# articulatory/articulatory

Measured on AMD Instinct MI355X. Metric: audio samples/sec (16 kHz) EMA->wav HiFi-CAR, batch 64, higher is better.
Workload: dtype fp32; 1 GPU; configs[2]: HiFi-CAR (e2w_hifigan_car.yaml generator) 13-dim pitch+EMA -> 16 kHz, batch 64/GPU, 10 s clips, 80 sequential chunks of 25 frames; batch_per_gpu=64, frames=2000, chunk_frames=25, weights=synthetic seed 1234 (articulatory_amd.utils.synth), parallelism=utterance-sharded x1, arithmetic=exact fp32 products (v_mfma_f32_32x32x2_f32), fp32 accumulate, gather=none

## Files before the change

articulatory_amd/csrc/hificar.hip:

```cpp
#include "hificar_kernels.hip.h"
#include "hificar_launch.h"
#include "hificar_backward.hip.h"
#include "hificar_disc_kernels.hip.h"
#include "hificar_bigru_kernels.hip.h"

#include "../../include/hificar.h"

#include <algorithm>
#include <queue>
#include <cmath>
#include <cstdarg>
#include <cstdio>
#include <cstring>
#include <functional>
#include <map>
#include <string>
#include <vector>

using namespace hificar;

static thread_local char g_err[1024] = "";

static int fail(int code, const char* fmt, ...) {
    va_list ap;
// ... 41 lines not shown
    int scale = 1;
    int cin = 0, cout = 0;
};

struct PlanKey {
    const ConvLayer* layers[6];
    int nseq, rows, zrep;
    int flags;
    bool operator<(const PlanKey& o) const { return memcmp(this, &o, sizeof(PlanKey)) < 0; }
};

struct ConvPlan {
    ConvShape shape;
    unsigned grid = 0;
    size_t lds = 0;
    std::string name;
    MultiConvParams conv = {};
    PairParams pair = {};
};

struct hificar_handle {
    hificar_config cfg;
    int arch = 0;
    std::vector<GBlockLayers> gb;
    int c_last = 0;
    bool finalized = false;
    int precision = HIFICAR_PREC_F32;
    bool profile_detail = false;
    bool use_pair = true;
    double mi1_penalty = 1.05;
    int pick_throughput = 0;
    bool pair_small = true;
    int ksplit = 1;
    int cf = 0;
    int cin_pad = 0;
    int hop = 1;
    int num_cus = 256;
    std::map<std::string, std::vector<int64_t>> expected;
    std::map<std::string, HostTensor> tensors;
    ConvLayer input_conv;
    std::vector<ConvLayer> ups;
    std::vector<ConvLayer> convs1;
    std::vector<ConvLayer> convs2;
    float* d_out_w = nullptr;
    float out_bias = 0.f;
    float* d_out_bias = nullptr;
    void* train = nullptr;
    void (*train_free)(hificar_handle*) = nullptr;
    float* d_mlp_w[5] = {nullptr, nullptr, nullptr, nullptr, nullptr};
    float* d_mlp_b[5] = {nullptr, nullptr, nullptr, nullptr, nullptr};
    float* d_spk_emb = nullptr;
    float* d_spk_w = nullptr;
    float* d_spk_b = nullptr;
    float* d_ph_emb = nullptr;
    float* d_phfc_w = nullptr;
    float* d_phfc_b = nullptr;
    std::vector<void*> allocs;
    char* d_zeros = nullptr;
    void* d_tab = nullptr;
    void* h_tab = nullptr;
    size_t tab_bytes = 0;
    hipEvent_t tab_copied = nullptr;
    struct StepSlot {
        hipEvent_t done = nullptr;
        bool used = false;
    };
// ... 27 lines not shown
    bool shared_chip = false;
    int ar_dual_min = 17, ar_dual_max = 62;
    hipStream_t ar_side = nullptr;
    hipEvent_t ar_ev[2] = {nullptr, nullptr};
    unsigned long long sched_up_seq = 0;
    hipEvent_t done_ev = nullptr;
    bool done_valid = false;
    hipStream_t done_stream = nullptr;
    struct Tap {
        float* dst;
        size_t cap;
    };
    std::map<std::string, Tap> taps;
    float* tap_scratch = nullptr;
    size_t tap_scratch_elems = 0;
    bool profiling = false;
    struct ProfRec {
        hipEvent_t e0, e1;
        std::string name;
        double flops, bytes;
    };
    std::vector<ProfRec> prof;
    hipStream_t prof_stream = nullptr;
};

static FILE* g_launch_log = nullptr;
static void read_env_switches(hificar_handle* h) {
    if (const char* e = getenv("HIFICAR_PROFILE_DETAIL")) h->profile_detail = atoi(e) != 0;
    if (const char* e = getenv("HIFICAR_LAUNCH_LOG")) {
        if (!g_launch_log && *e) g_launch_log = fopen(e, "a");
        if (g_launch_log) h->profile_detail = true;
    }
    if (const char* e = getenv("HIFICAR_KSPLIT")) h->ksplit = atoi(e);
    if (const char* e = getenv("HIFICAR_PAIR")) h->use_pair = atoi(e) != 0;
    if (const char* e = getenv("HIFICAR_PAIR_SMALL")) h->pair_small = atoi(e) != 0;
    if (const char* e = getenv("HIFICAR_AR_DUAL_MIN")) h->ar_dual_min = atoi(e);
    if (const char* e = getenv("HIFICAR_AR_DUAL_MAX")) h->ar_dual_max = atoi(e);
}

struct ProfScope {
    hificar_handle* h;
    hipStream_t s;
    hipEvent_t e0 = nullptr, e1 = nullptr;
    std::string name;
    double flops, bytes;
    ProfScope(hificar_handle* h_, hipStream_t s_, const std::string& n, double f, double b) : h(h_), s(s_), flops(f), bytes(b) {
        if (g_launch_log) {
            fprintf(g_launch_log, "%s\t%.0f\t%.0f\n", n.c_str(), f, b);
            fflush(g_launch_log);
        }
        if (!h->profiling) return;
        name = n;
        (void)hipEventCreate(&e0);
        (void)hipEventCreate(&e1);
        (void)hipEventRecord(e0, s);
    }
    ~ProfScope() {
        if (!h->profiling) return;
        (void)hipEventRecord(e1, s);
        h->prof.push_back({e0, e1, name, flops, bytes});
        h->prof_stream = s;
    }
};

static size_t round_up_sz(size_t x, size_t m) { return (x + m - 1) / m * m; }
static int arena_add(hificar_handle* h, size_t min_bytes);
// ... 708 lines not shown
        for (int t : lists[w]) tiles[pos++] = t;
    }
    start[G] = pos;
    *d_start = reinterpret_cast<int*>(a.d + a.used);
    *d_tiles = *d_start + n_start;
    a.used += take;
    HIP_TRY(hipMemcpyAsync(const_cast<int*>(*d_start), start, bytes, hipMemcpyHostToDevice, stream));
    ++h->sched_up_seq;
    return HIFICAR_OK;
}

static int enter_stream(hificar_handle* h, hipStream_t stream) {
    if (h->have_last_stream && h->last_stream != stream) {
        if (h->done_valid && h->done_stream == h->last_stream) {
            HIP_TRY(hipStreamWaitEvent(stream, h->done_ev, 0));
        } else {
            if (!h->xstream_ev) HIP_TRY(hipEventCreateWithFlags(&h->xstream_ev, hipEventDisableTiming));
            HIP_TRY(hipEventRecord(h->xstream_ev, h->last_stream));
            HIP_TRY(hipStreamWaitEvent(stream, h->xstream_ev, 0));
        }
    }
    h->done_valid = false;
    h->last_stream = stream;
    h->have_last_stream = true;
    return HIFICAR_OK;
}

struct TileCfg {
    int MI, WM, WN;
    int KS;
    int NB;
};
static size_t out_buf_bytes(const TileCfg& t) { return (size_t)t.KS * (t.WM * t.MI * 32) * (t.WN * t.NB * 32 + 4) * sizeof(float); }
constexpr int kNumTileCfgs = 15;
static const TileCfg kTileCfgs[kNumTileCfgs] = {{4, 1, 4, 1, 1}, {4, 2, 2, 1, 1}, {4, 4, 1, 1, 1}, {2, 2, 2, 1, 2}, {2, 4, 1, 1, 2},
                                                {2, 1, 4, 1, 2}, {2, 1, 4, 1, 1}, {2, 2, 2, 1, 1}, {2, 4, 1, 1, 1},
                                                {1, 1, 4, 1, 1}, {1, 2, 2, 1, 1}, {1, 4, 1, 1, 1}, {4, 1, 1, 4, 1}, {2, 1, 1, 4, 1}, {1, 1, 1, 4, 1}};

struct ConvIO {
    const char* xs;
    const float* res;
    float* y;
    char* ys;
    const float* mask_src = nullptr;
    float mask_slope = 0.f;
    long long x_seq_bytes = 0;
    int x_row_bytes = 0;
    int x_rows = 0;
    int x_up = 0;
    float x_slope = -1.f;
    const float* x_more[3] = {nullptr, nullptr, nullptr};
    int x_n = 1;
};

struct ConvRep {
    int n = 1;
    long long zs_x = 0, zs_w = 0, zs_y = 0, zs_b = 0;
};

static TileCfg pick_tile(const hificar_handle* h, const ConvLayer* const* layers, int nbr, int nseq, int rows, int zrep) {
    const ConvLayer& L0 = *layers[0];
    const bool f32 = h->precision == HIFICAR_PREC_F32;
    int halo_all = 0;
    for (int b = 0; b < nbr; ++b) halo_all = std::max(halo_all, layers[b]->off_max - layers[b]->off_min);
    TileCfg tc = {1, 4, 1, 1, 1};
    double best = 1e300;
    int nsteps_min = 1 << 30;
    for (int b = 0; b < nbr; ++b) nsteps_min = std::min(nsteps_min, layers[b]->ntaps * (L0.chunk16 / 16));
    for (int ti = 0; ti < kNumTileCfgs; ++ti) {
        const TileCfg& t = kTileCfgs[ti];
        const int TM = t.WM * t.MI * 32;
        const int chunk = L0.chunk16, RB = chunk * 4;
        if (t.NB == 2 && (f32 || L0.chunk16 == 16)) continue;
        const size_t obuf = (f32 && t.KS == 1) ? 0 : out_buf_bytes(t);
        if (2 * round_up_sz((size_t)(TM + halo_all) * RB, 1024) + obuf > 160 * 1024) continue;
        if (t.NB == 2) {
            bool ok = L0.n_blocks32 >= 2;
            for (int b = 0; b < nbr; ++b) ok = ok && (layers[b]->n_phase == 1 || layers[b]->nb32_per_phase % 2 == 0);
            if (!ok) continue;
        }
        if (t.KS == 4 && (h->ksplit == 0 || nsteps_min < 2)) continue;
        if (t.KS == 1 && h->ksplit == 2 && nsteps_min >= 2) continue;
        const long long tiles_per_branch = (long long)nseq * ((rows + TM - 1) / TM) * ((L0.n_blocks32 + t.WN * t.NB - 1) / (t.WN * t.NB));
        const long long total = tiles_per_branch * nbr * zrep;
        const int G = (int)std::min<long long>(total, h->num_cus);
        const int nchunks = L0.cin_pad / chunk;
        double total_cost = 0.0, heaviest = 0.0, lightest = 1e300, cb[3] = {0.0, 0.0, 0.0};
        for (int b = 0; b < nbr; ++b) {
            const double slab = f32 ? 8 * 64.0 : 3 * 32 / 0.75;
            double c = (double)layers[b]->ntaps * (L0.cin_pad / 16) * slab * t.MI * t.NB + 2500.0 + 400.0 * nchunks;
            if (t.KS == 4) {
                const int steps = layers[b]->ntaps * (chunk / 16);
                c = (double)((steps + 3) / 4) * nchunks * slab * t.MI + 4000.0 + 600.0 * nchunks;
            }
            total_cost += c * tiles_per_branch * zrep;
            heaviest = std::max(heaviest, c);
            lightest = std::min(lightest, c);
            cb[b] = c;
        }
        double worst = std::max(heaviest, total_cost / G);
        if (!h->shared_chip && total > G && total <= 4096) {
            std::sort(cb, cb + nbr, [](double x, double y) { return x > y; });
            std::priority_queue<double, std::vector<double>, std::greater<double>> load;
            for (int w = 0; w < G; ++w) load.push(0.0);
            worst = 0.0;
            for (int b = 0; b < nbr; ++b)
                for (long long i = 0; i < tiles_per_branch * zrep; ++i) {
                    const double v = load.top() + cb[b];
                    load.pop();
                    load.push(v);
                    worst = std::max(worst, v);
                }
        } else if (total % G != 0) {
            worst = std::max(worst, total_cost / G + 0.5 * lightest);
        }
        if (h->pick_throughput > 0 && total >= h->pick_throughput) worst = total_cost / h->num_cus;
        if (t.NB == 2) worst *= f32 ? (t.MI == 4 ? 0.95 : t.MI == 2 ? 0.975 : 1.02) : (t.MI == 2 ? 0.93 : 1.10);
        else if (t.MI < 4) worst *= f32 ? (t.MI == 2 ? 1.02 : h->mi1_penalty) : (t.MI == 2 ? 1.10 : 1.25);
        if (t.KS == 4) worst *= 1.05;
        if (worst < best * 0.98) {
            best = worst;
            tc = t;
        }
    }
    return tc;
}

static std::string plan_name(const hificar_handle* h, const ConvShape& s, const ConvLayer& L0, int nbr) {
    static const char* const family[] = {"conv_f32do_kernel", "conv_bf16x3_kernel", "conv_bf16x3nb_kernel", "conv_sk_f32_kernel", "conv_sk_bf16x3_kernel",
                                         "conv_pair_f32_kernel", "conv_pair_bf16x3_kernel"};
    char kname[96];
    int n = s.family == kConvSkF32 || s.family == kConvSkBf16x3 ? snprintf(kname, sizeof(kname), "%s<%d,%d>", family[s.family], s.mi, s.nc16)
                                                                : snprintf(kname, sizeof(kname), "%s<%d,%d,%d,%d>", family[s.family], s.mi, s.wm, s.wn, s.nc16);
    if (h->profile_detail) snprintf(kname + n, sizeof(kname) - n, "|%s x%d", L0.name.c_str(), nbr);
    return kname;
}

static int build_conv_plan(hificar_handle* h, const ConvLayer* const* layers, int nbr, int nseq, int rows, int zrep, hipStream_t stream, ConvPlan& pl) {
    const ConvLayer& L0 = *layers[0];
    const bool f32 = h->precision == HIFICAR_PREC_F32;
    MultiConvParams& mp = pl.conv;
    const TileCfg tc = pick_tile(h, layers, nbr, nseq, rows, zrep);
    int halo_all = 0;
    for (int b = 0; b < nbr; ++b) halo_all = std::max(halo_all, layers[b]->off_max - layers[b]->off_min);
    const int TM = tc.WM * tc.MI * 32, nc16 = L0.chunk16 / 16;
    const size_t buf_bytes = round_up_sz((size_t)(TM + halo_all) * L0.chunk16 * 4, 1024);
    const bool dout = f32 && tc.KS == 1;
    pl.shape = {dout ? kConvF32do : tc.KS == 4 ? (f32 ? kConvSkF32 : kConvSkBf16x3) : tc.NB == 2 ? kConvBf16x3nb : kConvBf16x3, tc.MI, tc.WM, tc.WN, nc16};
    pl.lds = 2 * buf_bytes + (dout ? 0 : out_buf_bytes(tc));
    mp.buf_bytes = (int)buf_bytes;
    mp.n_branches = nbr;
    mp.nseq_tiles = nseq * ((rows + TM - 1) / TM);
    mp.ngroups = (L0.n_blocks32 + tc.WN * tc.NB - 1) / (tc.WN * tc.NB);
    mp.total_tiles = nbr * zrep * mp.ngroups * mp.nseq_tiles;
    pl.grid = (unsigned)std::min(mp.total_tiles, h->num_cus);
    {
        double wbytes = 0.0;
        for (int b = 0; b < nbr; ++b) wbytes += 4.0 * layers[b]->cin_pad * layers[b]->cout_total * layers[b]->ntaps * zrep;
        const double abytes = 4.0 * nseq * rows * L0.cin_pad * nbr * zrep;
        mp.xcd_order = (mp.total_tiles <= h->num_cus && mp.total_tiles >= 16 && wbytes > 2.0 * abytes) ? 1 : 0;
    }
    mp.stage_cached = mp.ngroups > 2 ? 1 : 0;
    pl.name = plan_name(h, pl.shape, L0, nbr);
    TileLists lists;
    if (mp.total_tiles <= h->num_cus && nbr == 1 && zrep == 1 && mp.ngroups >= 2 && mp.nseq_tiles >= 8 && !h->shared_chip &&
        4.0 * L0.cin_pad * L0.cout_total * L0.ntaps > 6.0e6)
        lists = xcd_block_lists(mp.nseq_tiles, mp.ngroups, h->num_cus);
    if (!lists.empty()) {
        pl.grid = (unsigned)lists.size();
        mp.xcd_order = 0;
    } else if (mp.total_tiles > (int)pl.grid) {
        std::vector<double> costs((size_t)mp.total_tiles);
        const int tpb = mp.ngroups * mp.nseq_tiles * zrep;
        for (int b = 0; b < nbr; ++b)
            for (int i = 0; i < tpb; ++i) costs[(size_t)b * tpb + i] = layers[b]->ntaps + 1.0;
        lists = lpt_lists(costs, (int)pl.grid);
    }
    return lists.empty() ? HIFICAR_OK : upload_schedule(h, lists, mp.total_tiles, stream, &mp.sched_start, &mp.sched_tiles);
}

struct PairIOB {
    const float* xf;
    const char* xs;
    const float* res;
    float* y;
    char* ys;
};

static bool pair_small_tiles(const hificar_handle* h, int C, int k2, int nseq, int rows) {
    if (!h->pair_small || h->ksplit == 0 || C != 32 || h->precision != HIFICAR_PREC_F32 || nseq <= 0 || (long long)nseq * rows < 8000) return false;
    const int tmo = 4 * 4 * 32 - (k2 - 1);
    return 3LL * nseq * ((rows + tmo - 1) / tmo) < h->num_cus;
}

static bool pair_eligible(const hificar_handle* h, const ConvLayer& a, const ConvLayer& b, int nseq = 0, int rows = 0) {
    if (!(h->use_pair && a.d_w16c && b.d_w16c && a.d_w32c && b.d_w32c && a.cin == b.cin && a.ntaps >= 2 &&
          b.ntaps >= 2 && b.dilation == 1 && a.K == b.K))
        return false;
// ... 17 lines not shown
    const int C = l1[0]->cin;
    bool small = true;
    for (int b = 0; b < nbr; ++b) small = small && pair_small_tiles(h, C, l2[b]->ntaps, nseq, rows);
    const int MI = small ? 1 : 4, WM = C == 64 ? 2 : 4;
    const int TMc = WM * MI * 32, RB = C * 4;
    const bool f32 = h->precision == HIFICAR_PREC_F32;
    PairParams& pp = pl.pair;
    int halo_max = 0, tile = 0;
    for (int b = 0; b < nbr; ++b) {
        halo_max = std::max(halo_max, l1[b]->off_max - l1[b]->off_min);
        const int tmo = TMc - (l2[b]->ntaps - 1);
        pp.tiles_per_seq[b] = (rows + tmo - 1) / tmo;
        pp.tile_start[b] = tile;
        tile += nseq * pp.tiles_per_seq[b];
    }
    pp.tile_start[nbr] = tile;
    pp.n_branches = nbr;
    pp.nseq = nseq;
    pp.in_bytes = (int)round_up_sz((size_t)(TMc + halo_max) * RB, 1024);
    pp.ts_bytes = (int)std::max<size_t>((size_t)(TMc + 16) * RB, (size_t)TMc * (C + 4) * sizeof(float));
    pl.lds = (size_t)pp.in_bytes + pp.ts_bytes;
    if (pl.lds > 160 * 1024) return fail(HIFICAR_E_INVALID, "internal: pair kernel LDS too large (%zu)", pl.lds);
    pl.grid = (unsigned)std::min(tile, h->num_cus);
    pl.shape = {f32 ? kPairF32 : kPairBf16x3, MI, WM, 4 / WM, C / 16};
    pl.name = plan_name(h, pl.shape, *l1[0], nbr);
    if (tile <= (int)pl.grid) return HIFICAR_OK;
    std::vector<double> costs((size_t)tile);
    for (int b = 0; b < nbr; ++b)
        for (int i = pp.tile_start[b]; i < pp.tile_start[b + 1]; ++i) costs[i] = l1[b]->ntaps + l2[b]->ntaps + 2.0;
    return upload_schedule(h, lpt_lists(costs, (int)pl.grid), tile, stream, &pp.sched_start, &pp.sched_tiles);
}

static const ConvPlan* get_plan(hificar_handle* h, const ConvLayer* const* a, const ConvLayer* const* b, int nbr, int nseq, int rows, int zrep,
                                hipStream_t stream, int* rc) {
    *rc = HIFICAR_OK;
    PlanKey k = {{}, nseq, rows, zrep, (h->precision == HIFICAR_PREC_F32 ? 1 : 0) | (h->train ? 2 : 0) | (h->shared_chip ? 4 : 0) | (b ? 8 : 0)};
    for (int i = 0; i < nbr; ++i) k.layers[i] = a[i];
    for (int i = 0; b && i < nbr; ++i) k.layers[3 + i] = b[i];
    auto it = h->plans.find(k);
    if (it == h->plans.end()) {
        ConvPlan pl;
        if (h->plans.size() > 20000) *rc = evict_plans(h);
        if (*rc == HIFICAR_OK)
            *rc = b ? build_pair_plan(h, a, b, nbr, nseq, rows, stream, pl) : build_conv_plan(h, a, nbr, nseq, rows, zrep, stream, pl);
        if (*rc != HIFICAR_OK) return nullptr;
        it = h->plans.emplace(k, std::move(pl)).first;
    }
    return &it->second;
}

static int launch_conv(hificar_handle* h, const ConvLayer* const* layers, int nbr, int nseq, int rows, const ConvIO* io,
                              float slope_out, const Ragged& rg, hipStream_t stream, const ConvRep& zr = ConvRep()) {
    int rc;
    const ConvPlan* const pl = get_plan(h, layers, nullptr, nbr, nseq, rows, zr.n, stream, &rc);
    if (!pl) return rc;
    const int TM = pl->shape.wm * pl->shape.mi * 32;
    const ConvLayer& L0 = *layers[0];
    const bool f32 = h->precision == HIFICAR_PREC_F32;
    MultiConvParams mp = pl->conv;
    double flops = 0.0, bytes = 0.0;
    for (int b = 0; b < nbr; ++b) {
        const ConvLayer& Lb = *layers[b];
        if (Lb.n_blocks32 != L0.n_blocks32 || Lb.chunk16 != L0.chunk16 || Lb.cin_pad != L0.cin_pad)
            return fail(HIFICAR_E_INVALID, "internal: branch shape mismatch");
        fill_params(mp.p[b], Lb, rows, TM, io[b].res, io[b].y, rg);
        mp.p[b].xs = io[b].xs;
        mp.p[b].ys = io[b].ys;
        if (io[b].x_slope >= 0.f) {
            if (!f32) return fail(HIFICAR_E_INVALID, "internal: pre-activation input rows of %s outside the exact-fp32 layer-by-layer launches", Lb.name.c_str());
            if (io[b].x_n < 1 || io[b].x_n > 4) return fail(HIFICAR_E_INVALID, "internal: %d input streams of %s", io[b].x_n, Lb.name.c_str());
            mp.p[b].act_in = io[b].x_n;
            for (int q = 0; q + 1 < io[b].x_n; ++q) mp.p[b].xs_more[q] = reinterpret_cast<const char*>(io[b].x_more[q]);
            mp.p[b].slope_in = io[b].x_slope;
        }
        mp.p[b].mask_src = io[b].mask_src;
        mp.p[b].mask_slope = io[b].mask_slope;
        mp.p[b].x_seq_bytes = io[b].x_seq_bytes;
        mp.p[b].x_row_bytes = io[b].x_row_bytes;
        mp.p[b].x_rows = io[b].x_rows;
        if (io[b].x_up > 1) {
            if (rows % io[b].x_up != 0 || io[b].x_seq_bytes != 0 || io[b].x_row_bytes != 0)
                return fail(HIFICAR_E_INVALID, "internal: upsampled input rows of %s", Lb.name.c_str());
            mp.p[b].x_up = io[b].x_up;
            mp.p[b].x_up_rcp = (unsigned)(0x100000000ull / (unsigned)io[b].x_up) + 1u;
            mp.p[b].x_seq_bytes = (long long)(rows / io[b].x_up) * Lb.cin_pad * 4;
        }
        mp.p[b].zeros = h->d_zeros;
        mp.p[b].slope_out = slope_out;
        mp.p[b].cout_real = Lb.cout_pad;
        if (f32) mp.p[b].w16 = reinterpret_cast<const bf16x8*>(Lb.d_w32);
        const double pos = (double)nseq * rows;
        flops += 2.0 * pos * Lb.cin * Lb.cout * Lb.K * zr.n;
        bytes += 4.0 * (pos * Lb.cin_pad * (io[b].x_slope >= 0.f ? io[b].x_n : 1) / std::max(1, io[b].x_up) + pos * Lb.cout_total * ((io[b].res ? 1 : 0) + (io[b].y ? 1 : 0) + (io[b].ys ? 1 : 0)) +
                        (double)Lb.cin * Lb.cout * Lb.K);
    }
    mp.zrep = zr.n;
    mp.zs_x = zr.zs_x;
    mp.zs_w = zr.zs_w;
    mp.zs_y = zr.zs_y;
    mp.zs_b = zr.zs_b;
    ProfScope prof(h, stream, pl->name, flops, bytes);
    const hipError_t e = conv_launch(pl->shape, &mp, dim3(pl->grid, 1, 1), pl->lds, stream);
    if (e != hipSuccess) return fail(HIFICAR_E_HIP, "conv launch (%s, %s) failed: %s", L0.name.c_str(), pl->name.c_str(), hipGetErrorString(e));
    return HIFICAR_OK;
}

static int launch_pair(hificar_handle* h, const ConvLayer* const* l1, const ConvLayer* const* l2, int nbr, int nseq, int rows,
                              const PairIOB* io, float slope, const Ragged& rg, hipStream_t stream) {
    int rc;
    const ConvPlan* const pl = get_plan(h, l1, l2, nbr, nseq, rows, 1, stream, &rc);
    if (!pl) return rc;
    const int TMc = pl->shape.wm * pl->shape.mi * 32;
    const int C = l1[0]->cin;
    const bool f32 = h->precision == HIFICAR_PREC_F32;
    PairParams pp = pl->pair;
    double flops = 0.0, bytes = 0.0;
    for (int b = 0; b < nbr; ++b) {
        const ConvLayer& A = *l1[b];
        const ConvLayer& B = *l2[b];
        fill_params(pp.p1[b], A, rows, TMc, nullptr, nullptr, rg);
        fill_params(pp.p2[b], B, rows, TMc, io[b].res, io[b].y, rg);
        pp.p1[b].w16 = f32 ? reinterpret_cast<const bf16x8*>(A.d_w32c) : reinterpret_cast<const bf16x8*>(A.d_w16c);
        pp.p2[b].w16 = f32 ? reinterpret_cast<const bf16x8*>(B.d_w32c) : reinterpret_cast<const bf16x8*>(B.d_w16c);
        pp.p1[b].xs = io[b].xs;
        pp.p1[b].xf = io[b].xf;
        pp.p1[b].slope_in = slope;
        pp.p1[b].zeros = h->d_zeros;
// ... 183 lines not shown
        if (cfg.use_ar && (rc = emit_tap(h, "ar_feats", ws.xin, f32 ? h->cin_pad : -h->cin_pad, h->cf, cfg.ar_output, B, 1, f32 ? 0 : 1, stream, T)) != HIFICAR_OK)
            return rc;
    }
    const size_t tap_se = tapping ? stage_elems(h, B, T) : 0;
    const int nbk = cfg.n_blocks;
    int order[kMaxBlk];
    for (int j = 0; j < kMaxBlk; ++j) order[j] = j;
    std::sort(order, order + nbk, [&](int a, int b) { return cfg.resblock_kernel_sizes[a] > cfg.resblock_kernel_sizes[b]; });
    int max_d = 0;
    for (int j = 0; j < nbk; ++j) max_d = std::max(max_d, cfg.n_dilations[j]);
    int rows_of_launch = 0;
    const bool add_convs = cfg.use_additional_convs != 0;
    auto conv_n = [&](const ConvLayer* const* lay, int n, const ConvIO* io) -> int {
        for (int q0 = 0; q0 < n; q0 += 3) {
            const int r = launch_conv(h, lay + q0, std::min(3, n - q0), B, rows_of_launch, io + q0, cfg.lrelu_slope, rg, stream);
            if (r != HIFICAR_OK) return r;
        }
        return HIFICAR_OK;
    };

    const float* fin[kMaxBlk] = {ws.x[0], ws.x[1], ws.x[2], ws.x[3]};
    {
        char* xin_s = tp ? reinterpret_cast<char*>(tp->xin) : reinterpret_cast<char*>(ws.xin);
        char* h0_s = tp ? tp->h0_s : reinterpret_cast<char*>(ws.h0);
        char* xt_s[kMaxBlk] = {reinterpret_cast<char*>(ws.xt[0]), reinterpret_cast<char*>(ws.xt[1]), reinterpret_cast<char*>(ws.xt[2]),
                               reinterpret_cast<char*>(ws.xt[3])};
        {
            const ConvLayer* lay[1] = {&h->input_conv};
            float* y_tap = tap_wanted(h, "input_conv") ? h->tap_scratch + kMaxBlk * tap_se : nullptr;
            const ConvIO io[1] = {{xin_s, nullptr, y_tap, h0_s}};
            if ((rc = launch_conv(h, lay, 1, B, T, io, cfg.lrelu_slope, rg, stream)) != HIFICAR_OK) return rc;
            if (y_tap && (rc = emit_tap(h, "input_conv", y_tap, stage_pad(cfg, 0), 0, cfg.channels, B, T, 0, stream)) != HIFICAR_OK) return rc;
        }
        for (int i = 0; i < cfg.n_stages; ++i) {
            const char* up_in = h0_s;
            const bool fold_mrf = i > 0 && f32 && !tp;
            if (i > 0 && !fold_mrf) {
                MrfSplitParams mq;
                memset(&mq, 0, sizeof(mq));
                mq.x0 = fin[0];
                mq.x1 = nbk > 1 ? fin[1] : nullptr;
                mq.x2 = nbk > 2 ? fin[2] : nullptr;
                mq.x3 = nbk > 3 ? fin[3] : nullptr;
                mq.out = fin[0] == ws.xt[0] ? ws.x_s[0] : xt_s[0];
                if (tp) mq.out = tp->upin_s[i];
                mq.nin = nbk;
                mq.C = stage_pad(cfg, i);
                mq.rows = (long long)B * rows;
                mq.slope = cfg.lrelu_slope;
                mq.f32 = f32 ? 1 : 0;
                const long long units = mq.rows * (mq.C / 8);
                const unsigned blocks = (unsigned)std::min<long long>((units + 255) / 256, 8LL * h->num_cus);
                {
                    ProfScope prof(h, stream, "mrf_split_kernel", 0.0, 4.0 * mq.rows * mq.C * (nbk + 1));
                    hipLaunchKernelGGL(mrf_split_kernel, dim3(blocks), dim3(256), 0, stream, mq);
                }
                HIP_TRY(hipGetLastError());
                up_in = mq.out;
            }
            bool all_pairs = !tap_convs1 && !tp && add_convs;
            for (int j = 0; j < nbk && all_pairs; ++j)
                for (int d = 0; d < cfg.n_dilations[j]; ++d) {
                    const int ci = conv_index(h, i, j, d);
                    all_pairs = all_pairs && pair_eligible(h, h->convs1[ci], h->convs2[ci], B, rows * cfg.upsample_scales[i]);
                }
            {
                const ConvLayer* lay[1] = {&h->ups[i]};
                ConvIO io[1] = {{up_in, nullptr, ws.u, all_pairs ? nullptr : (tp ? tp->u_s[i] : ws.u_s)}};
                if (fold_mrf) {
                    io[0].xs = reinterpret_cast<const char*>(fin[0]);
// ... 25 lines not shown
                        if (d >= cfg.n_dilations[j]) continue;
                        const int ci = conv_index(h, i, j, d);
                        l1[n] = &h->convs1[ci];
                        l2[n] = &h->convs2[ci];
                        float* out_f = cur_f[j] == ws.x[j] ? ws.xt[j] : ws.x[j];
                        iop[n] = {cur_f[j], nullptr, cur_f[j], out_f, nullptr};
                        cur_f[j] = out_f;
                        ++n;
                    }
                    for (int q0 = 0; q0 < n; q0 += 3)
                        if ((rc = launch_pair(h, l1 + q0, l2 + q0, std::min(3, n - q0), B, rows, iop + q0, cfg.lrelu_slope, rg, stream)) != HIFICAR_OK) return rc;
                    for (int j = 0; j < nbk; ++j)
                        if (d < cfg.n_dilations[j] && (rc = tap_block(j, d, cur_f[j])) != HIFICAR_OK) return rc;
                }
                for (int j = 0; j < nbk; ++j) fin[j] = cur_f[j];
                continue;
            }
            float* xres[kMaxBlk] = {ws.x[0], ws.x[1], ws.x[2], ws.x[3]};
            if (tp && i + 1 == cfg.n_stages)
                for (int j = 0; j < nbk; ++j) xres[j] = tp->fin[j];
            for (int j = 0; j < nbk; ++j) fin[j] = xres[j];
            const char* u_act = tp ? tp->u_s[i] : ws.u_s;
            const char* cur_s[kMaxBlk] = {u_act, u_act, u_act, u_act};
            for (int d = 0; d < max_d; ++d) {
                const ConvLayer* l1[kMaxBlk];
                const ConvLayer* l2[kMaxBlk];
                ConvIO io1[kMaxBlk], io2[kMaxBlk];
                PairIOB iop[kMaxBlk];
                int jn[kMaxBlk];
                char* pair_out[kMaxBlk];
                char* lbl_out[kMaxBlk];
                int n = 0;
                bool fuse = add_convs;
                for (int oj = 0; oj < nbk; ++oj) {
                    const int j = order[oj];
                    if (d >= cfg.n_dilations[j]) continue;
                    const int ci = conv_index(h, i, j, d);
                    l1[n] = &h->convs1[ci];
                    l2[n] = add_convs ? &h->convs2[ci] : nullptr;
                    fuse = fuse && !tap_convs1 && !tp && pair_eligible(h, *l1[n], *l2[n], B, rows);
                    const bool last = d + 1 == cfg.n_dilations[j];
                    pair_out[n] = cur_s[j] == ws.x_s[j] ? xt_s[j] : ws.x_s[j];
                    char* mid = cur_s[j] == xt_s[j] ? ws.x_s[j] : xt_s[j];
                    lbl_out[n] = mid == xt_s[j] ? ws.x_s[j] : xt_s[j];
                    if (tp) {
                        mid = tp->xt_s[i][j][d];
                        lbl_out[n] = tp->x_s[i][j][d];
                    }
                    io1[n] = {cur_s[j], nullptr, tap_convs1 ? h->tap_scratch + (size_t)n * tap_se : nullptr, mid};
                    io2[n] = {mid, d == 0 ? ws.u : xres[j], xres[j], last ? nullptr : lbl_out[n]};
                    if (!add_convs) {
                        char* nxt = tp ? tp->x_s[i][j][d] : pair_out[n];
                        io1[n] = {cur_s[j], d == 0 ? ws.u : xres[j], xres[j], last ? nullptr : nxt};
                        lbl_out[n] = nxt;
                    }
                    iop[n] = {nullptr, cur_s[j], d == 0 ? ws.u : xres[j], xres[j], last ? nullptr : pair_out[n]};
                    jn[n] = j;
                    ++n;
                }
                if (fuse) {
                    for (int q0 = 0; q0 < n; q0 += 3)
                        if ((rc = launch_pair(h, l1 + q0, l2 + q0, std::min(3, n - q0), B, rows, iop + q0, cfg.lrelu_slope, rg, stream)) != HIFICAR_OK) return rc;
                } else if (!add_convs) {
                    rows_of_launch = rows;
                    if ((rc = conv_n(l1, n, io1)) != HIFICAR_OK) return rc;
                } else {
                    rows_of_launch = rows;
                    if ((rc = conv_n(l1, n, io1)) != HIFICAR_OK) return rc;
                    if (tap_convs1)
                        for (int q = 0; q < n; ++q)
                            if ((rc = emit_tap(h, "blocks." + std::to_string(i * nbk + jn[q]) + ".convs1." + std::to_string(d), io1[q].y, Cp, 0, Cs,
                                               B, rows, 0, stream)) != HIFICAR_OK)
                                return rc;
                    if ((rc = conv_n(l2, n, io2)) != HIFICAR_OK) return rc;
                }
                for (int q = 0; q < n; ++q)
                    if ((rc = tap_block(jn[q], d, xres[jn[q]])) != HIFICAR_OK) return rc;
                for (int q = 0; q < n; ++q) cur_s[jn[q]] = fuse ? pair_out[q] : lbl_out[q];
            }
        }
    }
    if (cfg.use_ph_loss && cond.ph_out) {
        PhHeadParams pq;
        memset(&pq, 0, sizeof(pq));
        pq.x0 = fin[0];
        pq.x1 = nbk > 1 ? fin[1] : nullptr;
        pq.x2 = nbk > 2 ? fin[2] : nullptr;
        pq.x3 = nbk > 3 ? fin[3] : nullptr;
        pq.nin = nbk;
        pq.w = h->d_phfc_w;
        pq.bias = h->d_phfc_b;
        pq.out = cond.ph_out;
        pq.C = stage_channels(cfg, cfg.n_stages);
        pq.Cp = stage_pad(cfg, cfg.n_stages);
        pq.L = rows;
        pq.T = cond.ph_out_T;
        pq.hop = h->hop;
        pq.num_ph = cfg.num_ph;
        pq.seq_len = seq_len;
        pq.len_const = seq_len ? -1 : (T_valid < T ? T_valid : -1);
        ProfScope prof(h, stream, "ph_head_kernel", 2.0 * B * T_valid * (double)pq.C * cfg.num_ph, 4.0 * B * (double)rows * pq.Cp * nbk);
        hipLaunchKernelGGL(ph_head_kernel, dim3(T_valid, B), dim3(256), 0, stream, pq);
        HIP_TRY(hipGetLastError());
    }
    return launch_output_conv(h, fin, nbk, stage_pad(cfg, cfg.n_stages), rows, B, T, out, out_bstride, seq_len, rg, slots, stream);
}

// ... 399 lines not shown
```

articulatory_amd/csrc/hificar_conv.hip.h:

```cpp
#pragma once
#include <hip/hip_runtime.h>
#include <stdint.h>
#include <type_traits>

namespace hificar {

typedef float f32x2 __attribute__((ext_vector_type(2)));
typedef float f32x4 __attribute__((ext_vector_type(4)));
typedef unsigned u32x4_t __attribute__((ext_vector_type(4)));
typedef float f32x16 __attribute__((ext_vector_type(16)));
typedef __bf16 bf16x4 __attribute__((ext_vector_type(4)));
typedef __bf16 bf16x8 __attribute__((ext_vector_type(8)));

constexpr int kMaxPhase = 8;
constexpr int kMaxTaps = 16;

struct ConvParams {
    const bf16x8* w16;
    const float* bias;
    const float* res;
    const float* mask_src;
    float mask_slope;
    float* y;
    const float* xf;
// ... 31 lines not shown
    asm volatile("s_load_dword %0, %1, 0x0\n\ts_waitcnt lgkmcnt(0)" : "=s"(v) : "s"(p) : "memory");
    return v;
}

__device__ __forceinline__ void scalar_load_2i32(const int* p, int& a, int& b) {
    long long v;
    asm volatile("s_load_dwordx2 %0, %1, 0x0\n\ts_waitcnt lgkmcnt(0)" : "=s"(v) : "s"(p) : "memory");
    a = (int)v;
    b = (int)(v >> 32);
}

__device__ __forceinline__ bool is_ragged(const ConvParams& p) { return p.seq_len != nullptr || p.len_const >= 0; }

__device__ __forceinline__ int seq_rows(const ConvParams& p, int seq) {
    if (!is_ragged(p)) return p.L;
    const int n = (p.seq_len ? scalar_load_i32(p.seq_len + __builtin_amdgcn_readfirstlane(seq)) : p.len_const) - p.len_f0;
    return min(max(n, 0), p.len_max) * p.len_mul;
}

struct MultiConvParams {
    ConvParams p[3];
    int n_branches;
    int nseq_tiles;
    int ngroups;
    int total_tiles;
    int buf_bytes;
    const int* sched_start;
    const int* sched_tiles;
    int zrep;
    long long zs_x, zs_w, zs_y, zs_b;
    unsigned long long* trace;
    int xcd_order;
    int stage_cached;
};


#ifdef HIFICAR_TRACE
__device__ unsigned long long g_trace_realtime[2][1024];
__device__ unsigned long long g_trace_rt_slots[4][64];
#define HIFICAR_STAMP(slot)                                                                            \
    do {                                                                                               \
        if (mp.trace && lane == 0 && (wave == 0 || wave == kFirstLoader) && (slot) < 64)               \
            mp.trace[((size_t)blockIdx.x * 2 + (wave ? 1 : 0)) * 64 + (slot)] = __builtin_amdgcn_s_memtime(); \
        if (mp.trace && lane == 0 && wave == 0 && ((slot) == 0 || (slot) == 63) && blockIdx.x < 1024)  \
            g_trace_realtime[(slot) == 63][blockIdx.x] = __builtin_amdgcn_s_memrealtime();             \
        if (mp.trace && lane == 0 && wave == 0 && (slot) < 64 && blockIdx.x < 4)                       \
            g_trace_rt_slots[blockIdx.x][(slot)] = __builtin_amdgcn_s_memrealtime();                   \
    } while (0)
#else
#define HIFICAR_STAMP(slot) do { } while (0)
#endif

__device__ __forceinline__ float lrelu(float v, float slope) { return v >= 0.f ? v : v * slope; }


template <int I, int NDS, int NVMEM, int NMFMA>
__device__ __forceinline__ void pin_slab_slot() {
    if constexpr (I < NMFMA) {
        constexpr int NMEM = NDS + NVMEM;
        constexpr int lo = NMEM * I / NMFMA, hi = NMEM * (I + 1) / NMFMA;
        constexpr int ds = (hi < NDS ? hi : NDS) - (lo < NDS ? lo : NDS);
        constexpr int vm = (hi - lo) - ds;
        __builtin_amdgcn_sched_group_barrier(0x008, 1, 0);
        if constexpr (ds > 0) __builtin_amdgcn_sched_group_barrier(0x100, ds, 0);
        if constexpr (vm > 0) __builtin_amdgcn_sched_group_barrier(0x020, vm, 0);
        pin_slab_slot<I + 1, NDS, NVMEM, NMFMA>();
// ... 38 lines not shown
    const int nchunks = mp.p[0].cin / CH;
    const int tiles_per_branch = mp.ngroups * mp.nseq_tiles;
    const int buf_bytes = mp.buf_bytes;

    struct Tile {
        int b, z, ng, seq, t0;
    };
    auto decode = [&](int tile) {
        Tile T;
        const unsigned ut = (unsigned)tile, tpb = (unsigned)tiles_per_branch, zr = (unsigned)mp.zrep, nst = (unsigned)mp.nseq_tiles;
        const unsigned bz = ut / tpb;
        const unsigned b = bz / zr;
        T.b = (int)b;
        T.z = (int)(bz - b * zr);
        const unsigned rem = ut - bz * tpb;
        const unsigned ng = rem / nst;
        T.ng = (int)ng;
        const unsigned m = rem - ng * nst;
        const unsigned tps = (unsigned)mp.p[0].tiles_per_seq;
        const unsigned seq = m / tps;
        T.seq = (int)seq;
        T.t0 = (int)((m - seq * tps) * (unsigned)TM);
        return T;
    };

    constexpr int TN = WN * NB * 32;
    constexpr int OP = TN + 4;
    int sched_lo = 0, sched_hi = 0;
    if (mp.sched_start) scalar_load_2i32(mp.sched_start + blockIdx.x, sched_lo, sched_hi);
    const int my_rounds = mp.sched_start ? sched_hi - sched_lo
                                         : (mp.total_tiles - (int)blockIdx.x + (int)gridDim.x - 1) / (int)gridDim.x;
    auto tile_of = [&](int it) {
        int i = it;
        if ((blockIdx.x & 1) && my_rounds >= 3 && it >= my_rounds - 2) i = it == my_rounds - 1 ? my_rounds - 2 : my_rounds - 1;
        if (mp.sched_start) return scalar_load_i32(mp.sched_tiles + sched_lo + i);
        if (mp.xcd_order) {
            const int x = (int)blockIdx.x & 7, l = (int)blockIdx.x >> 3;
            const int base = mp.total_tiles >> 3, rem = mp.total_tiles & 7;
            return x * base + min(x, rem) + l;
        }
        return (int)blockIdx.x + (my_rounds - 1 - i) * (int)gridDim.x;
    };
    auto nxt = [&](int i) {
        if (is_ragged(mp.p[0]))
            while (i < my_rounds) {
                const Tile T = decode(tile_of(i));
                if (T.t0 < seq_rows(mp.p[T.b], T.seq)) break;
                ++i;
            }
        return i;
    };
    const float* O = reinterpret_cast<const float*>(smem_b + 2 * buf_bytes);
    auto write_out = [&](const Tile& T, int ltid, int nthr) {
        const ConvParams& p = mp.p[T.b];
        const int vc_base = T.ng * TN;
        const int width = min(TN, p.n_blocks32 * 32 - vc_base);
        const int w8 = width >> 3;
        const int rpp = nthr / w8;
        const int rr = ltid / w8;
        const int c8 = (ltid - rr * w8) * 8;
        const bool lane_on = rr < rpp;
        const size_t seq_base = (size_t)T.seq * p.L;
        const float slope_out = p.slope_out;
        const int rows = min(TM, seq_rows(p, T.seq) - T.t0);
        const float* const bias_z = p.bias + (size_t)T.z * mp.zs_b;
        float* const y_z = p.y ? p.y + (size_t)T.z * mp.zs_y : nullptr;
        char* const ys_z = p.ys ? p.ys + (size_t)T.z * mp.zs_y * 4 : nullptr;
// ... 374 lines not shown
            for (int r = 0; r < 16; ++r) off16[r] = voff + (int)((8 * (r >> 2) + (r & 3)) * pitch_b);
            const float slope_out = p.slope_out, mask_slope = p.mask_slope;
            auto pass = [&](auto HR, auto HM, auto HY, auto HS) {
                constexpr bool kRes = decltype(HR)::value, kMask = decltype(HM)::value, kY = decltype(HY)::value, kYs = decltype(HS)::value;
                auto fetch1 = [&](int mi, int r, float (&rs)[16], float (&mk)[16]) {
                    if constexpr (kRes) rs[r] = __builtin_bit_cast(float, __builtin_amdgcn_raw_buffer_load_b32(rsrc_of(b_res, has_res, mi), off16[r], 0, 0));
                    if constexpr (kMask) mk[r] = __builtin_bit_cast(float, __builtin_amdgcn_raw_buffer_load_b32(rsrc_of(b_mask, has_mask, mi), off16[r], 0, 0));
                };
                auto finish = [&](int mi, int r, const float (&rs)[16], const float (&mk)[16]) {
                    float o = acc[0][mi][r] + bias_l;
                    if constexpr (kMask) o *= mk[r] > 0.f ? 1.f : mask_slope;
                    if constexpr (kRes) o += rs[r];
                    if constexpr (kY) __builtin_amdgcn_raw_buffer_store_b32(__builtin_bit_cast(unsigned, o), rsrc_of(b_y, has_y, mi), off16[r], 0, kAux);
                    if constexpr (kYs) __builtin_amdgcn_raw_buffer_store_b32(__builtin_bit_cast(unsigned, __builtin_amdgcn_fmed3f(o, o * slope_out, __builtin_inff())), rsrc_of(b_ys, has_ys, mi), off16[r], 0, kAux);
                };
                {
                    constexpr int G2 = MI >= 2 ? 2 : 1;
#pragma unroll
                    for (int m0 = 0; m0 < MI; m0 += G2) {
                        float rs[G2][16], mk[G2][16];
                        if constexpr (kRes || kMask) {
#pragma unroll
                            for (int mm = 0; mm < G2; ++mm)
#pragma unroll
                                for (int r = 0; r < 16; ++r) fetch1(m0 + mm, r, rs[mm], mk[mm]);
                        }
#pragma unroll
                        for (int mm = 0; mm < G2; ++mm)
#pragma unroll
                            for (int r = 0; r < 16; ++r) finish(m0 + mm, r, rs[mm], mk[mm]);
                    }
                }
            };
            constexpr std::true_type Y{};
            constexpr std::false_type N{};
            if (has_mask) {
                pass(Y, Y, Y, Y);
                return;
            }
            if (has_res) {
                if (has_y && has_ys) pass(Y, N, Y, Y);
                else if (has_y) pass(Y, N, Y, N);
                else pass(Y, N, N, Y);
            } else {
                if (has_y && has_ys) pass(N, N, Y, Y);
                else if (has_y) pass(N, N, Y, N);
                else pass(N, N, N, Y);
            }
        }
    };
    auto bias_of = [&](const Tile& T) {
        const int nb = (T.ng * WN + wn) * NB;
        return (mp.p[T.b].bias + (size_t)T.z * mp.zs_b)[(nb < mp.p[T.b].n_blocks32 ? nb : 0) * 32 + li];
    };
    int j = 0;
    int last = -1;
    HIFICAR_STAMP(0);
    if constexpr (KS == 4) {
        const int ks = cw;
        constexpr int LOG_NC = NC16 == 4 ? 2 : NC16 == 2 ? 1 : 0;
        for (int it = nxt(0); it < my_rounds; it = nxt(it + 1)) {
            last = it;
            const Tile T = decode(tile_of(it));
            const ConvParams& p = mp.p[T.b];
            const int nb = T.ng;
            const int phase = (int)((unsigned)nb / (unsigned)p.nb32_per_phase);
            const int roff0 = __builtin_amdgcn_readfirstlane(p.tap_off0[phase] - p.off_min);
            const int tap_step = p.tap_step;
// ... 718 lines not shown
```

Before: 39.77 million samples/s.

## Fuse MRF branch averaging into last resblock conv via LDS accumulation

Adds a summing mode for the last multi-branch resblock conv of each non-final stage. The MRF branches of a tile group are scheduled consecutively on the same workgroup and accumulate their residual outputs in LDS. The last branch writes the mean with leaky-ReLU applied directly as the next upsample input, which skips the per-branch output writes and the separate MRF mean/split pass. The cost is extra LDS, a restriction to fp32 non-ksplit tiles, and fewer parallel tiles since branches are serialised per workgroup. A cost model picks the mode only when it is estimated to be no worse.

```diff
diff --git a/articulatory_amd/csrc/hificar.hip b/articulatory_amd/csrc/hificar.hip
--- a/articulatory_amd/csrc/hificar.hip
+++ b/articulatory_amd/csrc/hificar.hip
@@ -97,6 +97,7 @@
     int pick_throughput = 0;
     bool pair_small = true;
     int ksplit = 1;
+    int mrf_sum = -1;
     int cf = 0;
     int cin_pad = 0;
     int hop = 1;
@@ -190,6 +191,7 @@
         if (g_launch_log) h->profile_detail = true;
     }
     if (const char* e = getenv("HIFICAR_KSPLIT")) h->ksplit = atoi(e);
+    if (const char* e = getenv("HIFICAR_MRF_SUM")) h->mrf_sum = atoi(e) != 0 ? 1 : 0;
     if (const char* e = getenv("HIFICAR_PAIR")) h->use_pair = atoi(e) != 0;
     if (const char* e = getenv("HIFICAR_PAIR_SMALL")) h->pair_small = atoi(e) != 0;
     if (const char* e = getenv("HIFICAR_AR_DUAL_MIN")) h->ar_dual_min = atoi(e);
@@ -964,6 +966,7 @@
     int NB;
 };
 static size_t out_buf_bytes(const TileCfg& t) { return (size_t)t.KS * (t.WM * t.MI * 32) * (t.WN * t.NB * 32 + 4) * sizeof(float); }
+static size_t sum_buf_bytes(const TileCfg& t) { return (size_t)t.WM * t.WN * t.MI * 16 * 64 * sizeof(float); }
 constexpr int kNumTileCfgs = 15;
 static const TileCfg kTileCfgs[kNumTileCfgs] = {{4, 1, 4, 1, 1}, {4, 2, 2, 1, 1}, {4, 4, 1, 1, 1}, {2, 2, 2, 1, 2}, {2, 4, 1, 1, 2},
                                                 {2, 1, 4, 1, 2}, {2, 1, 4, 1, 1}, {2, 2, 2, 1, 1}, {2, 4, 1, 1, 1},
@@ -985,12 +988,20 @@
     int x_n = 1;
 };
 
+struct ConvSum {
+    float* dst;
+    float slope;
+    int pos[3];
+    bool used = false;
+};
+
 struct ConvRep {
     int n = 1;
     long long zs_x = 0, zs_w = 0, zs_y = 0, zs_b = 0;
 };
 
-static TileCfg pick_tile(const hificar_handle* h, const ConvLayer* const* layers, int nbr, int nseq, int rows, int zrep) {
+static TileCfg pick_tile(const hificar_handle* h, const ConvLayer* const* layers, int nbr, int nseq, int rows, int zrep, int sum_n = 0,
+                         double* cost_out = nullptr) {
     const ConvLayer& L0 = *layers[0];
     const bool f32 = h->precision == HIFICAR_PREC_F32;
     int halo_all = 0;
@@ -1004,7 +1015,8 @@
         const int TM = t.WM * t.MI * 32;
         const int chunk = L0.chunk16, RB = chunk * 4;
         if (t.NB == 2 && (f32 || L0.chunk16 == 16)) continue;
-        const size_t obuf = (f32 && t.KS == 1) ? 0 : out_buf_bytes(t);
+        if (sum_n && !(f32 && t.KS == 1 && t.NB == 1)) continue;
+        const size_t obuf = (f32 && t.KS == 1) ? (sum_n ? sum_buf_bytes(t) : 0) : out_buf_bytes(t);
         if (2 * round_up_sz((size_t)(TM + halo_all) * RB, 1024) + obuf > 160 * 1024) continue;
         if (t.NB == 2) {
             bool ok = L0.n_blocks32 >= 2;
@@ -1014,7 +1026,7 @@
         if (t.KS == 4 && (h->ksplit == 0 || nsteps_min < 2)) continue;
         if (t.KS == 1 && h->ksplit == 2 && nsteps_min >= 2) continue;
         const long long tiles_per_branch = (long long)nseq * ((rows + TM - 1) / TM) * ((L0.n_blocks32 + t.WN * t.NB - 1) / (t.WN * t.NB));
-        const long long total = tiles_per_branch * nbr * zrep;
+        const long long total = tiles_per_branch * (sum_n ? 1 : nbr) * zrep;
         const int G = (int)std::min<long long>(total, h->num_cus);
         const int nchunks = L0.cin_pad / chunk;
         double total_cost = 0.0, heaviest = 0.0, lightest = 1e300, cb[3] = {0.0, 0.0, 0.0};
@@ -1030,13 +1042,19 @@
             lightest = std::min(lightest, c);
             cb[b] = c;
         }
+        int nunit = nbr;
+        if (sum_n) {
+            cb[0] = cb[0] + cb[1] + cb[2];
+            heaviest = lightest = cb[0];
+            nunit = 1;
+        }
         double worst = std::max(heaviest, total_cost / G);
         if (!h->shared_chip && total > G && total <= 4096) {
-            std::sort(cb, cb + nbr, [](double x, double y) { return x > y; });
+            std::sort(cb, cb + nunit, [](double x, double y) { return x > y; });
             std::priority_queue<double, std::vector<double>, std::greater<double>> load;
             for (int w = 0; w < G; ++w) load.push(0.0);
             worst = 0.0;
-            for (int b = 0; b < nbr; ++b)
+            for (int b = 0; b < nunit; ++b)
                 for (long long i = 0; i < tiles_per_branch * zrep; ++i) {
                     const double v = load.top() + cb[b];
                     load.pop();
@@ -1055,6 +1073,7 @@
             tc = t;
         }
     }
+    if (cost_out) *cost_out = best;
     return tc;
 }
 
@@ -1068,18 +1087,29 @@
     return kname;
 }
 
-static int build_conv_plan(hificar_handle* h, const ConvLayer* const* layers, int nbr, int nseq, int rows, int zrep, hipStream_t stream, ConvPlan& pl) {
+static int build_conv_plan(hificar_handle* h, const ConvLayer* const* layers, int nbr, int nseq, int rows, int zrep, hipStream_t stream, ConvPlan& pl,
+                           const int* sum_pos = nullptr) {
     const ConvLayer& L0 = *layers[0];
     const bool f32 = h->precision == HIFICAR_PREC_F32;
     MultiConvParams& mp = pl.conv;
-    const TileCfg tc = pick_tile(h, layers, nbr, nseq, rows, zrep);
+    double cost = 0.0;
+    TileCfg tc = pick_tile(h, layers, nbr, nseq, rows, zrep, 0, &cost);
+    bool sum = false;
+    if (sum_pos && f32 && tc.KS == 1 && zrep == 1 && nbr >= 2) {
+        double cost_sum = 0.0;
+        const TileCfg ts = pick_tile(h, layers, nbr, nseq, rows, zrep, nbr, &cost_sum);
+        if (cost_sum < 1e299 && (h->mrf_sum == 1 || cost_sum <= cost * 1.005)) {
+            sum = true;
+            tc = ts;
+        }
+    }
     int halo_all = 0;
     for (int b = 0; b < nbr; ++b) halo_all = std::max(halo_all, layers[b]->off_max - layers[b]->off_min);
     const int TM = tc.WM * tc.MI * 32, nc16 = L0.chunk16 / 16;
     const size_t buf_bytes = round_up_sz((size_t)(TM + halo_all) * L0.chunk16 * 4, 1024);
     const bool dout = f32 && tc.KS == 1;
     pl.shape = {dout ? kConvF32do : tc.KS == 4 ? (f32 ? kConvSkF32 : kConvSkBf16x3) : tc.NB == 2 ? kConvBf16x3nb : kConvBf16x3, tc.MI, tc.WM, tc.WN, nc16};
-    pl.lds = 2 * buf_bytes + (dout ? 0 : out_buf_bytes(tc));
+    pl.lds = 2 * buf_bytes + (dout ? (sum ? sum_buf_bytes(tc) : 0) : out_buf_bytes(tc));
     mp.buf_bytes = (int)buf_bytes;
     mp.n_branches = nbr;
     mp.nseq_tiles = nseq * ((rows + TM - 1) / TM);
@@ -1095,7 +1125,25 @@
     mp.stage_cached = mp.ngroups > 2 ? 1 : 0;
     pl.name = plan_name(h, pl.shape, L0, nbr);
     TileLists lists;
-    if (mp.total_tiles <= h->num_cus && nbr == 1 && zrep == 1 && mp.ngroups >= 2 && mp.nseq_tiles >= 8 && !h->shared_chip &&
+    if (sum) {
+        const int ngr = mp.ngroups * mp.nseq_tiles;
+        pl.grid = (unsigned)std::min(ngr, h->num_cus);
+        mp.xcd_order = 0;
+        mp.sum_n = nbr;
+        int by_pos[3] = {0, 1, 2};
+        std::sort(by_pos, by_pos + nbr, [&](int a, int b) { return sum_pos[a] < sum_pos[b]; });
+        for (int q = 0; q < nbr; ++q) mp.sum_pos[by_pos[q]] = q;
+        double gcost = 0.0;
+        for (int b = 0; b < nbr; ++b) gcost += layers[b]->ntaps + 1.0;
+        const TileLists glists = lpt_lists(std::vector<double>((size_t)ngr, gcost), (int)pl.grid);
+        lists.resize(glists.size());
+        for (size_t w = 0; w < glists.size(); ++w) {
+            std::vector<int> gl = glists[w];
+            if ((w & 1) && gl.size() >= 3) std::swap(gl[gl.size() - 1], gl[gl.size() - 2]);
+            for (int gi : gl)
+                for (int q = 0; q < nbr; ++q) lists[w].push_back(by_pos[q] * ngr + gi);
+        }
+    } else if (mp.total_tiles <= h->num_cus && nbr == 1 && zrep == 1 && mp.ngroups >= 2 && mp.nseq_tiles >= 8 && !h->shared_chip &&
         4.0 * L0.cin_pad * L0.cout_total * L0.ntaps > 6.0e6)
         lists = xcd_block_lists(mp.nseq_tiles, mp.ngroups, h->num_cus);
     if (!lists.empty()) {
@@ -1179,9 +1227,10 @@
 }
 
 static const ConvPlan* get_plan(hificar_handle* h, const ConvLayer* const* a, const ConvLayer* const* b, int nbr, int nseq, int rows, int zrep,
-                                hipStream_t stream, int* rc) {
+                                hipStream_t stream, int* rc, const int* sum_pos = nullptr) {
     *rc = HIFICAR_OK;
-    PlanKey k = {{}, nseq, rows, zrep, (h->precision == HIFICAR_PREC_F32 ? 1 : 0) | (h->train ? 2 : 0) | (h->shared_chip ? 4 : 0) | (b ? 8 : 0)};
+    PlanKey k = {{}, nseq, rows, zrep,
+                 (h->precision == HIFICAR_PREC_F32 ? 1 : 0) | (h->train ? 2 : 0) | (h->shared_chip ? 4 : 0) | (b ? 8 : 0) | (sum_pos ? 16 : 0)};
     for (int i = 0; i < nbr; ++i) k.layers[i] = a[i];
     for (int i = 0; b && i < nbr; ++i) k.layers[3 + i] = b[i];
     auto it = h->plans.find(k);
@@ -1189,7 +1238,7 @@
         ConvPlan pl;
         if (h->plans.size() > 20000) *rc = evict_plans(h);
         if (*rc == HIFICAR_OK)
-            *rc = b ? build_pair_plan(h, a, b, nbr, nseq, rows, stream, pl) : build_conv_plan(h, a, nbr, nseq, rows, zrep, stream, pl);
+            *rc = b ? build_pair_plan(h, a, b, nbr, nseq, rows, stream, pl) : build_conv_plan(h, a, nbr, nseq, rows, zrep, stream, pl, sum_pos);
         if (*rc != HIFICAR_OK) return nullptr;
         it = h->plans.emplace(k, std::move(pl)).first;
     }
@@ -1197,10 +1246,12 @@
 }
 
 static int launch_conv(hificar_handle* h, const ConvLayer* const* layers, int nbr, int nseq, int rows, const ConvIO* io,
-                              float slope_out, const Ragged& rg, hipStream_t stream, const ConvRep& zr = ConvRep()) {
+                              float slope_out, const Ragged& rg, hipStream_t stream, const ConvRep& zr = ConvRep(), ConvSum* sum = nullptr) {
     int rc;
-    const ConvPlan* const pl = get_plan(h, layers, nullptr, nbr, nseq, rows, zr.n, stream, &rc);
+    const ConvPlan* const pl = get_plan(h, layers, nullptr, nbr, nseq, rows, zr.n, stream, &rc, sum ? sum->pos : nullptr);
     if (!pl) return rc;
+    const bool summing = sum && pl->conv.sum_n > 0;
+    if (sum) sum->used = summing;
     const int TM = pl->shape.wm * pl->shape.mi * 32;
     const ConvLayer& L0 = *layers[0];
     const bool f32 = h->precision == HIFICAR_PREC_F32;
@@ -1210,9 +1261,11 @@
         const ConvLayer& Lb = *layers[b];
         if (Lb.n_blocks32 != L0.n_blocks32 || Lb.chunk16 != L0.chunk16 || Lb.cin_pad != L0.cin_pad)
             return fail(HIFICAR_E_INVALID, "internal: branch shape mismatch");
-        fill_params(mp.p[b], Lb, rows, TM, io[b].res, io[b].y, rg);
+        float* const y_b = summing ? nullptr : io[b].y;
+        char* const ys_b = summing ? nullptr : io[b].ys;
+        fill_params(mp.p[b], Lb, rows, TM, io[b].res, y_b, rg);
         mp.p[b].xs = io[b].xs;
-        mp.p[b].ys = io[b].ys;
+        mp.p[b].ys = ys_b;
         if (io[b].x_slope >= 0.f) {
             if (!f32) return fail(HIFICAR_E_INVALID, "internal: pre-activation input rows of %s outside the exact-fp32 layer-by-layer launches", Lb.name.c_str());
             if (io[b].x_n < 1 || io[b].x_n > 4) return fail(HIFICAR_E_INVALID, "internal: %d input streams of %s", io[b].x_n, Lb.name.c_str());
@@ -1238,8 +1291,13 @@
         if (f32) mp.p[b].w16 = reinterpret_cast<const bf16x8*>(Lb.d_w32);
         const double pos = (double)nseq * rows;
         flops += 2.0 * pos * Lb.cin * Lb.cout * Lb.K * zr.n;
-        bytes += 4.0 * (pos * Lb.cin_pad * (io[b].x_slope >= 0.f ? io[b].x_n : 1) / std::max(1, io[b].x_up) + pos * Lb.cout_total * ((io[b].res ? 1 : 0) + (io[b].y ? 1 : 0) + (io[b].ys ? 1 : 0)) +
+        bytes += 4.0 * (pos * Lb.cin_pad * (io[b].x_slope >= 0.f ? io[b].x_n : 1) / std::max(1, io[b].x_up) + pos * Lb.cout_total * ((io[b].res ? 1 : 0) + (y_b ? 1 : 0) + (ys_b ? 1 : 0)) +
                         (double)Lb.cin * Lb.cout * Lb.K);
+    }
+    if (summing) {
+        mp.sum_dst = sum->dst;
+        mp.sum_slope = sum->slope;
+        bytes += 4.0 * nseq * rows * L0.cout_total;
     }
     mp.zrep = zr.n;
     mp.zs_x = zr.zs_x;
@@ -1489,10 +1547,16 @@
             if ((rc = launch_conv(h, lay, 1, B, T, io, cfg.lrelu_slope, rg, stream)) != HIFICAR_OK) return rc;
             if (y_tap && (rc = emit_tap(h, "input_conv", y_tap, stage_pad(cfg, 0), 0, cfg.channels, B, T, 0, stream)) != HIFICAR_OK) return rc;
         }
+        bool sum_ok = f32 && !tp && !tapping && h->mrf_sum != 0 && nbk >= 2 && nbk <= 3;
+        for (int j = 1; j < nbk; ++j) sum_ok = sum_ok && cfg.n_dilations[j] == cfg.n_dilations[0];
+        const char* mrf_mean = nullptr;
         for (int i = 0; i < cfg.n_stages; ++i) {
             const char* up_in = h0_s;
-            const bool fold_mrf = i > 0 && f32 && !tp;
-            if (i > 0 && !fold_mrf) {
+            const bool summed = mrf_mean != nullptr;
+            const bool fold_mrf = i > 0 && f32 && !tp && !summed;
+            if (summed) up_in = mrf_mean;
+            mrf_mean = nullptr;
+            if (i > 0 && !fold_mrf && !summed) {
                 MrfSplitParams mq;
                 memset(&mq, 0, sizeof(mq));
                 mq.x0 = fin[0];
@@ -1584,6 +1648,16 @@
                 char* lbl_out[kMaxBlk];
                 int n = 0;
                 bool fuse = add_convs;
+                auto conv_last = [&](const ConvLayer* const* lay, int nl, const ConvIO* io) -> int {
+                    if (!(sum_ok && d + 1 == max_d && i + 1 < cfg.n_stages && nl == nbk)) return conv_n(lay, nl, io);
+                    ConvSum cs;
+                    cs.dst = reinterpret_cast<float*>(lbl_out[0]);
+                    cs.slope = cfg.lrelu_slope;
+                    for (int q = 0; q < nl; ++q) cs.pos[q] = jn[q];
+                    const int r = launch_conv(h, lay, nl, B, rows_of_launch, io, cfg.lrelu_slope, rg, stream, ConvRep(), &cs);
+                    if (r == HIFICAR_OK && cs.used) mrf_mean = lbl_out[0];
+                    return r;
+                };
                 for (int oj = 0; oj < nbk; ++oj) {
                     const int j = order[oj];
                     if (d >= cfg.n_dilations[j]) continue;
@@ -1615,7 +1689,7 @@
                         if ((rc = launch_pair(h, l1 + q0, l2 + q0, std::min(3, n - q0), B, rows, iop + q0, cfg.lrelu_slope, rg, stream)) != HIFICAR_OK) return rc;
                 } else if (!add_convs) {
                     rows_of_launch = rows;
-                    if ((rc = conv_n(l1, n, io1)) != HIFICAR_OK) return rc;
+                    if ((rc = conv_last(l1, n, io1)) != HIFICAR_OK) return rc;
                 } else {
                     rows_of_launch = rows;
                     if ((rc = conv_n(l1, n, io1)) != HIFICAR_OK) return rc;
@@ -1624,7 +1698,7 @@
                             if ((rc = emit_tap(h, "blocks." + std::to_string(i * nbk + jn[q]) + ".convs1." + std::to_string(d), io1[q].y, Cp, 0, Cs,
                                                B, rows, 0, stream)) != HIFICAR_OK)
                                 return rc;
-                    if ((rc = conv_n(l2, n, io2)) != HIFICAR_OK) return rc;
+                    if ((rc = conv_last(l2, n, io2)) != HIFICAR_OK) return rc;
                 }
                 for (int q = 0; q < n; ++q)
                     if ((rc = tap_block(jn[q], d, xres[jn[q]])) != HIFICAR_OK) return rc;
diff --git a/articulatory_amd/csrc/hificar_conv.hip.h b/articulatory_amd/csrc/hificar_conv.hip.h
--- a/articulatory_amd/csrc/hificar_conv.hip.h
+++ b/articulatory_amd/csrc/hificar_conv.hip.h
@@ -87,6 +87,10 @@
     unsigned long long* trace;
     int xcd_order;
     int stage_cached;
+    int sum_n;
+    int sum_pos[3];
+    float sum_slope;
+    float* sum_dst;
 };
 
 
@@ -191,7 +195,7 @@
                                          : (mp.total_tiles - (int)blockIdx.x + (int)gridDim.x - 1) / (int)gridDim.x;
     auto tile_of = [&](int it) {
         int i = it;
-        if ((blockIdx.x & 1) && my_rounds >= 3 && it >= my_rounds - 2) i = it == my_rounds - 1 ? my_rounds - 2 : my_rounds - 1;
+        if ((blockIdx.x & 1) && my_rounds >= 3 && it >= my_rounds - 2 && !(DOUT && mp.sum_n)) i = it == my_rounds - 1 ? my_rounds - 2 : my_rounds - 1;
         if (mp.sched_start) return scalar_load_i32(mp.sched_tiles + sched_lo + i);
         if (mp.xcd_order) {
             const int x = (int)blockIdx.x & 7, l = (int)blockIdx.x >> 3;
@@ -632,8 +636,51 @@
                     }
                 }
             };
+            auto sum_pass = [&](auto POS) {
+                constexpr int kPos = decltype(POS)::value;
+                int lane_s = lane, n_sum = mp.sum_n;
+                asm volatile("" : "+v"(lane_s), "+s"(n_sum));
+                float* const S = reinterpret_cast<float*>(smem_b + 2 * buf_bytes) + (cw * 16 * MI) * 64 + lane_s;
+                const float nf = (float)n_sum, slope_sum = mp.sum_slope;
+                const unsigned long long b_sum = kPos == 2 ? uni64((unsigned long long)(mp.sum_dst + first)) : 0ull;
+                constexpr int G2 = 1;
+#pragma unroll
+                for (int m0 = 0; m0 < MI; m0 += G2) {
+                    float rs[G2][16], sv[G2][16];
+#pragma unroll
+                    for (int mm = 0; mm < G2; ++mm)
+#pragma unroll
+                        for (int r = 0; r < 16; ++r) {
+                            rs[mm][r] = __builtin_bit_cast(float, __builtin_amdgcn_raw_buffer_load_b32(rsrc_of(b_res, has_res, m0 + mm), off16[r], 0, 0));
+                            if constexpr (kPos > 0) sv[mm][r] = S[((m0 + mm) * 16 + r) * 64];
+                        }
+#pragma unroll
+                    for (int mm = 0; mm < G2; ++mm)
+#pragma unroll
+                        for (int r = 0; r < 16; ++r) {
+                            float o = acc[0][m0 + mm][r] + bias_l;
+                            o += rs[mm][r];
+                            if constexpr (kPos == 0) {
+                                S[((m0 + mm) * 16 + r) * 64] = o;
+                            } else if constexpr (kPos == 1) {
+                                S[((m0 + mm) * 16 + r) * 64] = sv[mm][r] + o;
+                            } else {
+                                const float m = (sv[mm][r] + o) / nf;
+                                __builtin_amdgcn_raw_buffer_store_b32(__builtin_bit_cast(unsigned, __builtin_amdgcn_fmed3f(m, m * slope_sum, __builtin_inff())),
+                                                                      rsrc_of(b_sum, true, m0 + mm), off16[r], 0, kAux);
+                            }
+                        }
+                }
+            };
             constexpr std::true_type Y{};
             constexpr std::false_type N{};
+            if (mp.sum_n) {
+                const int pos = mp.sum_pos[T.b];
+                if (pos == 0) sum_pass(std::integral_constant<int, 0>{});
+                else if (pos + 1 < mp.sum_n) sum_pass(std::integral_constant<int, 1>{});
+                else sum_pass(std::integral_constant<int, 2>{});
+                return;
+            }
             if (has_mask) {
                 pass(Y, Y, Y, Y);
                 return;
```

Result: no change. 40.07 million samples/s, median of 6 (+0.8%).
